# real-stanford/semantic-abstraction

Hardware: AMD Instinct MI355X
Metric: scenes/sec (relevancy+3D-UNet infer), 480x480x16-label x128^3 (higher is better)
Workload: dtype f16 (MFMA operands, fp32 accumulate; UNet hi/lo-split = fp32-equivalent); 1 GPU; end-to-end relevancy->fusion->OVSSC per scene: 480x480 RGB-D, 16 labels, ViT-B/16, 'ours' saliency config (2448 tile forwards), 128^3 voxels, 80000 input points; scene-sharded; arch=ViT-B/16, unet_precision=exact, tile_chunk_streams=1, scenes_per_gpu=26, parallelism=scene-shard x1, mode=throughput

## Files before the change

semantic-abstraction_amd/csrc/unet.hip:

```cpp
#include "semabs_common.h"

__device__ __forceinline__ int xcd_remap(int vb, int nb) {
    const int q = nb >> 3, r = nb & 7, x = vb & 7, k = vb >> 3;
    return (x < r ? x * (q + 1) : r * (q + 1) + (x - r) * q) + k;
}
__device__ __forceinline__ int xcd_persistent_tile(int vb, int G, int it, int total) {
    if (G & 7) { const long t = (long)it * G + vb; return t < total ? (int)t : -1; }
    const int x = vb & 7, j = vb >> 3, g8 = G >> 3;
    const int q = total >> 3, r = total & 7;
    const int lo = x < r ? x * (q + 1) : r * (q + 1) + (x - r) * q, cnt = q + (x < r ? 1 : 0);
    const long o = (long)it * g8 + j;
    return o < cnt ? lo + (int)o : -1;
}


template <int HID, int COUT>
__global__ __launch_bounds__(256, 2) void k_point_mlp(const float* __restrict__ xyz, const float* __restrict__ feat,
                                                   const float* __restrict__ w1, const float* __restrict__ b1,
                                                   const float* __restrict__ w2, const float* __restrict__ b2,
                                                   const float* __restrict__ w3, const float* __restrict__ b3,
                                                   float* __restrict__ out, int P, long N) {
    extern __shared__ __attribute__((aligned(16))) char smem[];
    float* sw2 = reinterpret_cast<float*>(smem);
    float* sw3 = sw2 + HID * HID;
// ... 901 lines not shown
    auto lds_barrier = [&]() { asm volatile("s_waitcnt lgkmcnt(0)\n\ts_barrier" ::: "memory"); };
    auto brick_of = [&](int it) { return xcd_persistent_tile((int)blockIdx.x, (int)gridDim.x, it, total); };
    if (producer) {
        int it = 0, brick = brick_of(0);
        if (brick >= 0) produce(brick, 0);
        lds_barrier();
        int buf = 0;
        for (; brick >= 0; buf ^= 1) {
            const int next = brick_of(++it);
            if (next >= 0 && !CONV16_ABL(a.ablate == 2 || a.ablate >= 4)) produce(next, buf ^ 1);
            lds_barrier();
            brick = next;
        }
    } else {
        load_weights();
        lds_barrier();
        int buf = 0, it = 0;
        for (int brick = brick_of(0); brick >= 0; brick = brick_of(++it), buf ^= 1) {
            if (!CONV16_ABL(a.ablate == 1)) consume(brick, buf);
            lds_barrier();
        }
        if (a.stats) flush_stats();
        if (GNB && a.gnb_bits) conv_absmax_commit(a.gnb_bits, amax);
    }
}

#define SEMABS_CONV_GENERIC 256
#define SEMABS_CONV_PACKED 512
#ifdef SEMABS_TUNING
static int g_conv16_ablate = 0;
static long long* g_conv_trace = nullptr;
static int g_brick_persist = 0;
static int g_convt_no_line = 0;
extern "C" int semabs_conv_tune(int key, long long value) {
    if (key == 0) g_conv16_ablate = (int)value & 7;
    else if (key == 1) g_conv_trace = reinterpret_cast<long long*>(value);
    else if (key == 2) g_brick_persist = (int)value;
    else if (key == 3) g_convt_no_line = (int)value;
    return SEMABS_OK;
}
#endif

static int conv16_lds_launch(const ConvArgs& a_in, int f32, hipStream_t s) {
    ConvArgs a = a_in;
#ifdef SEMABS_TUNING
    a.ablate = g_conv16_ablate;
#endif
    if (f32) {
        constexpr int T0 = 4;
        const size_t lds = (size_t)(((T0 + 2) * C16_H1 * C16_H2 * 8 + 127) / 128 * 128) * 2 * 2 * 2 * 2;
        const long total = (long)a.B * (a.I0 / T0) * (a.I1 / C16_T1) * (a.I2 / C16_T2);
        long nb = semabs_stream_cus(s); if (nb > total) nb = total;
        if (a.gnb_coef) {
            static SemabsLdsAttr attrg;
            semabs_ensure_lds(&k_conv16_lds<true, T0, true>, (int)(lds + 32 * 192), attrg);
            hipLaunchKernelGGL((k_conv16_lds<true, T0, true>), dim3((unsigned)nb), dim3(512), lds + (size_t)a.B * 192, s, a);
            SEMABS_CHECK_LAUNCH();
            return SEMABS_OK;
        }
        if (a.occ) {
            static SemabsLdsAttr attrs;
            semabs_ensure_lds(&k_conv16_lds<true, T0, false, true>, (int)lds, attrs);
            hipLaunchKernelGGL((k_conv16_lds<true, T0, false, true>), dim3((unsigned)nb), dim3(512), lds, s, a);
            SEMABS_CHECK_LAUNCH();
            return SEMABS_OK;
        }
        static SemabsLdsAttr attr;
        semabs_ensure_lds(&k_conv16_lds<true, T0>, (int)lds, attr);
        hipLaunchKernelGGL((k_conv16_lds<true, T0>), dim3((unsigned)nb), dim3(512), lds, s, a);
    } else {
        constexpr int T0 = 8;
// ... 349 lines not shown
    }
    BRICK_STAMP(7);
}

template <bool F32, int CW, int NB, bool ONE, bool PERSIST, int TX = 16, bool GNB = false>
static int conv_brick_launch_p(const ConvArgs& a, hipStream_t s) {
    const size_t lds = (size_t)((6 * C16_H1 * (TX + 2) * 8 + 127) / 128 * 128) * (CW / 8) * 2 * (F32 ? 2 : 1);
    static int per_cu = 0;
    if (!per_cu) {
        (void)hipFuncSetAttribute(reinterpret_cast<const void*>(&k_conv_brick<F32, CW, NB, ONE, PERSIST, TX, GNB>), hipFuncAttributeMaxDynamicSharedMemorySize, (int)lds);
        int n = 0;
        if (hipOccupancyMaxActiveBlocksPerMultiprocessor(&n, k_conv_brick<F32, CW, NB, ONE, PERSIST, TX, GNB>, 512, lds) != hipSuccess || n < 1) n = 1;
        per_cu = n;
    }
    const long total = (long)(a.I0 / 4) * (a.I1 / C16_T1) * (a.I2 / TX) * a.B * (a.Cout / (NB * 16));
    SEMABS_REQUIRE(total < (1L << 30), "conv brick: too many tiles");
    long nwg = total;
    if (PERSIST) { nwg = (long)semabs_stream_cus(s) * per_cu; if (nwg > total) nwg = total; }
    ConvArgs at = a;
#ifdef SEMABS_TUNING
    at.trace = g_conv_trace;
#endif
    hipLaunchKernelGGL((k_conv_brick<F32, CW, NB, ONE, PERSIST, TX, GNB>), dim3((unsigned)nwg), dim3(512), lds, s, at, (int)total);
    SEMABS_CHECK_LAUNCH();
    return SEMABS_OK;
}
template <bool F32, int CW, int NB, bool ONE>
static int conv_brick_launch_t(const ConvArgs& a, hipStream_t s) {
#ifdef SEMABS_TUNING
    if (g_brick_persist) return conv_brick_launch_p<F32, CW, NB, ONE, true>(a, s);
#endif
    return conv_brick_launch_p<F32, CW, NB, ONE, false>(a, s);
}
static int conv_brick_launch(const ConvArgs& a, int f32, hipStream_t s) {
    if (a.gnb_coef) {
        if (a.Cin == 32) return conv_brick_launch_p<true, 32, 2, true, false, 16, true>(a, s);
        return conv_brick_launch_p<true, 32, 2, false, false, 16, true>(a, s);
    }
    if (a.I2 % C16_T2 != 0) {
        return f32 ? conv_brick_launch_p<true, 32, 2, false, false, 8>(a, s) : conv_brick_launch_p<false, 32, 2, false, false, 8>(a, s);
    }
    const long bricks = (long)a.B * (a.I0 / 4) * (a.I1 / C16_T1) * (a.I2 / C16_T2);
    if (a.Cout == 16) {
        if (a.Cin == 32) return f32 ? conv_brick_launch_t<true, 32, 1, true>(a, s) : conv_brick_launch_t<false, 32, 1, true>(a, s);
        return f32 ? conv_brick_launch_t<true, 32, 1, false>(a, s) : conv_brick_launch_t<false, 32, 1, false>(a, s);
    }
    const bool nb4 = a.Cout % 64 == 0 && bricks * (a.Cout / 64) >= 512;
    if (a.Cin == 16) {
        if (nb4) return f32 ? conv_brick_launch_t<true, 16, 4, true>(a, s) : conv_brick_launch_t<false, 16, 4, true>(a, s);
        return f32 ? conv_brick_launch_t<true, 16, 2, true>(a, s) : conv_brick_launch_t<false, 16, 2, true>(a, s);
    }
    if (a.Cin == 32) {
        if (nb4) return f32 ? conv_brick_launch_t<true, 32, 4, true>(a, s) : conv_brick_launch_t<false, 32, 4, true>(a, s);
        return f32 ? conv_brick_launch_t<true, 32, 2, true>(a, s) : conv_brick_launch_t<false, 32, 2, true>(a, s);
    }
    if (nb4) return f32 ? conv_brick_launch_t<true, 32, 4, false>(a, s) : conv_brick_launch_t<false, 32, 4, false>(a, s);
    return f32 ? conv_brick_launch_t<true, 32, 2, false>(a, s) : conv_brick_launch_t<false, 32, 2, false>(a, s);
}

__global__ void k_conv_finish(float* __restrict__ y, const float* __restrict__ bias, const float* __restrict__ resid, long n4, int C, int relu) {
    const long i = (long)blockIdx.x * blockDim.x + threadIdx.x;
    if (i >= n4) return;
    float4 v = *reinterpret_cast<float4*>(y + i * 4);
    if (bias) { const float4 b = *reinterpret_cast<const float4*>(bias + (i * 4) % C); v.x += b.x; v.y += b.y; v.z += b.z; v.w += b.w; }
    if (resid) { const float4 r = *reinterpret_cast<const float4*>(resid + i * 4); v.x += r.x; v.y += r.y; v.z += r.z; v.w += r.w; }
    if (relu == 1) { v.x = fmaxf(v.x, 0.f); v.y = fmaxf(v.y, 0.f); v.z = fmaxf(v.z, 0.f); v.w = fmaxf(v.w, 0.f); }
    else if (relu == 2) { v.x = v.x > 0.f ? v.x : 0.01f * v.x; v.y = v.y > 0.f ? v.y : 0.01f * v.y; v.z = v.z > 0.f ? v.z : 0.01f * v.z; v.w = v.w > 0.f ? v.w : 0.01f * v.w; }
    *reinterpret_cast<float4*>(y + i * 4) = v;
}

static int conv_launch(const ConvArgs& a_in, int f32, hipStream_t s) {
    ConvArgs a = a_in;
    const long Mtot = (long)a.B * a.M0 * a.M1 * a.M2;
    a.ksplit = 1;
    if (f32 && a.os == 1 && a.Cout % 64 == 0 && a.Cin % 32 == 0 && a.ntaps == 27 && Mtot <= 16384) {
        const long slices = semabs_cdiv(Mtot, 4 * 32) * (a.Cout / 64);
        int ks = (int)(2048 / (slices > 0 ? slices : 1));
        if (ks > 27) ks = 27;
        if (ks >= 3) {
            a.ksplit = ks;
// ... 50 lines not shown
    const bool bricks = !(act_flags & SEMABS_CONV_GENERIC);
    int rc = conv_common_checks(x, w_hi, w_lo, y, Cin, Cout, act_f32);
    if (rc) return rc;
    SEMABS_REQUIRE(ksize == 1 || ksize == 3, "semabs_conv3d: kernel size must be 1 or 3");
    SEMABS_REQUIRE((gn_scale == nullptr) == (gn_shift == nullptr), "semabs_conv3d: gn_scale and gn_shift go together");
    ConvArgs a;
    a.x = x; a.y = y; a.w_hi = (const f16*)w_hi; a.w_lo = (const f16*)w_lo; a.gn_scale = gn_scale; a.gn_shift = gn_shift;
    a.bias = bias; a.resid = resid; a.B = B; a.I0 = D0; a.I1 = D1; a.I2 = D2; a.O0 = D0; a.O1 = D1; a.O2 = D2;
    a.M0 = D0; a.M1 = D1; a.M2 = D2; a.os = 1; a.is = 1; a.op0 = a.op1 = a.op2 = 0; a.Cin = Cin; a.Cout = Cout; a.relu = relu;
    a.ntaps = ksize * ksize * ksize;
    a.Kp = ((a.ntaps * Cin + 31) / 32) * 32;
    a.stats = nullptr; a.ablate = 0; a.trace = nullptr; a.wp_hi = nullptr; a.wp_lo = nullptr; a.ncls = 0;
    if (act_flags & SEMABS_CONV_PACKED) {
        a.wp_hi = a.w_hi + (long)Cout * a.Kp;
        if (w_lo) a.wp_lo = a.w_lo + (long)Cout * a.Kp;
    }
    int t = 0;
    for (int kd = 0; kd < ksize; ++kd)
        for (int kh = 0; kh < ksize; ++kh)
            for (int kw = 0; kw < ksize; ++kw, ++t) { a.td0[t] = kd - ksize / 2; a.td1[t] = kh - ksize / 2; a.td2[t] = kw - ksize / 2; }
    SEMABS_REQUIRE(relu == 0 || relu == 1 || (relu == 2 && ksize == 1), "semabs_conv3d: relu must be 0, 1, or 2 (LeakyReLU, ksize 1 only)");
    SEMABS_REQUIRE(!out_sums || (out_groups > 0 && Cout % out_groups == 0), "semabs_conv3d_stats: Cout must be a multiple of out_groups");
    bool fused = false;
    if (bricks && ksize == 3 && Cin == 16 && Cout == 16 && D0 % 8 == 0 && D1 % C16_T1 == 0 && D2 % C16_T2 == 0 && (long)D0 * D1 * D2 * 16 < (1L << 31)) {
        if (out_sums && out_groups == 8) { a.stats = out_sums; fused = true; }
        a.occ = occ;
        rc = conv16_lds_launch(a, act_f32, (hipStream_t)stream);
    } else if (occ) {
        semabs_set_error("semabs_conv3d_sparse_stats: the occupancy bitmap is read by the 16 -> 16 level-0 kernel only (D0 % 8, D1 % 8, D2 % 16 == 0)");
        return SEMABS_EINVAL;
    } else if (bricks && ksize == 3 && (Cout % 32 == 0 || (Cout == 16 && Cin % 32 == 0 && D2 % C16_T2 == 0)) && (Cin == 16 || Cin % 32 == 0) && relu != 2 &&
               D0 % 4 == 0 && D1 % C16_T1 == 0 && (D2 % C16_T2 == 0 || (D2 % 8 == 0 && Cin % 32 == 0))) {
        if (out_sums && out_groups == 8 && Cout >= 32) { a.stats = out_sums; fused = true; }
        rc = conv_brick_launch(a, act_f32, (hipStream_t)stream);
    } else {
        rc = conv_launch(a, act_f32, (hipStream_t)stream);
    }
    if (rc == SEMABS_OK && out_sums && !fused) rc = semabs_gn_stats(y, out_sums, B, (long)D0 * D1 * D2, Cout, out_groups, act_f32, stream);
    return rc;
}
extern "C" int semabs_conv3d(const void* x, const void* w_hi, const void* w_lo, void* y, const float* gn_scale, const float* gn_shift,
                             const float* bias, const void* resid, int B, int D0, int D1, int D2, int Cin, int Cout, int ksize,
                             int relu, int act_f32, void* stream) {
    return conv3d_impl(x, w_hi, w_lo, y, gn_scale, gn_shift, bias, resid, B, D0, D1, D2, Cin, Cout, ksize, relu, act_f32, nullptr, 0, stream);
}
extern "C" int semabs_conv3d_stats(const void* x, const void* w_hi, const void* w_lo, void* y, const float* gn_scale, const float* gn_shift,
                                   const float* bias, const void* resid, int B, int D0, int D1, int D2, int Cin, int Cout, int ksize,
                                   int relu, int act_f32, double* out_sums, int out_groups, void* stream) {
    SEMABS_REQUIRE(out_sums, "semabs_conv3d_stats: out_sums is null");
    return conv3d_impl(x, w_hi, w_lo, y, gn_scale, gn_shift, bias, resid, B, D0, D1, D2, Cin, Cout, ksize, relu, act_f32, out_sums, out_groups, stream);
}

extern "C" int semabs_conv3d_sparse_stats(const void* x, const unsigned int* occ, const void* w_hi, const void* w_lo, void* y, const float* gn_scale, const float* gn_shift,
                                          const float* bias, const void* resid, int B, int D0, int D1, int D2, int Cin, int Cout, int ksize,
                                          int relu, int act_f32, double* out_sums, int out_groups, void* stream) {
    SEMABS_REQUIRE(out_sums && occ, "semabs_conv3d_sparse_stats: out_sums / occ is null");
    SEMABS_REQUIRE(!(act_f32 & SEMABS_CONV_GENERIC), "semabs_conv3d_sparse_stats: the generic kernel reads the whole volume");
    return conv3d_impl(x, w_hi, w_lo, y, gn_scale, gn_shift, bias, resid, B, D0, D1, D2, Cin, Cout, ksize, relu, act_f32, out_sums, out_groups, stream, occ);
}

static int conv3d_gnbwd_route(int B, int D0, int D1, int D2, int Cin, int Cout, int G, bool have_add) {
    if (B <= 0 || G <= 0) return 0;
    if (B <= 32 && Cin == 16 && Cout == 16 && D0 % 8 == 0 && D1 % C16_T1 == 0 && D2 % C16_T2 == 0 && (long)D0 * D1 * D2 * 16 < (1L << 31) && 16 % G == 0) return 1;
    if (!have_add && Cin % 32 == 0 && Cout % 32 == 0 && Cout % G == 0 && (Cout / G) % 4 == 0 && D0 % 4 == 0 && D1 % C16_T1 == 0 && D2 % C16_T2 == 0) return 2;
    return 0;
}
extern "C" int semabs_conv3d_gnbwd_supported(int B, int D0, int D1, int D2, int Cin, int Cout, int G, int have_add1, int* ok) {
// ... 623 lines not shown
```

Baseline: 8.675 scenes/s.

## Add persistent warp-specialized producer/consumer conv kernel for wide-input fp32 UNet layers

Adds a new persistent 3D conv kernel in which four producer waves stage GroupNorm-applied, hi/lo-split f16 halo tiles into double-buffered LDS per 16-channel unit, while four consumer waves run MFMA with register-prefetched weights. For NB=2 it uses a dy-reuse schedule that shares each loaded input row across three kernel rows. It routes fp32 convs with Cin>=64 to it by default. The aim is to overlap global loads with MFMA and to cut redundant LDS and input traffic, at the cost of much more code, heavier register pressure and a new correctness surface.

```diff
diff --git a/semantic-abstraction_amd/csrc/unet.hip b/semantic-abstraction_amd/csrc/unet.hip
--- a/semantic-abstraction_amd/csrc/unet.hip
+++ b/semantic-abstraction_amd/csrc/unet.hip
@@ -957,11 +957,13 @@
 static long long* g_conv_trace = nullptr;
 static int g_brick_persist = 0;
 static int g_convt_no_line = 0;
+static int g_conv_units = 0;
 extern "C" int semabs_conv_tune(int key, long long value) {
     if (key == 0) g_conv16_ablate = (int)value & 7;
     else if (key == 1) g_conv_trace = reinterpret_cast<long long*>(value);
     else if (key == 2) g_brick_persist = (int)value;
     else if (key == 3) g_convt_no_line = (int)value;
+    else if (key == 4) g_conv_units = (int)value;
     return SEMABS_OK;
 }
 #endif
@@ -1377,6 +1379,408 @@
 #endif
     return conv_brick_launch_p<F32, CW, NB, ONE, false>(a, s);
 }
+
+template <int NB>
+__global__ __launch_bounds__(512) void k_conv_units(ConvArgs a, int total) {
+    constexpr bool DY = NB == 2;
+    constexpr int T0 = 4, H0 = T0 + 2, HX = C16_H2, HALO = H0 * C16_H1 * HX, NSTEPS = 14;
+    constexpr int PLANE = (HALO * 8 + 127) / 128 * 128;
+    constexpr int BUF_EL = PLANE * 2 * 2;
+    constexpr int ZPAD = HALO * 8;
+    static_assert(PLANE - ZPAD >= 8, "no room for the zero slot");
+    extern __shared__ __attribute__((aligned(16))) char smem[];
+    const int tid = threadIdx.x, lane = tid & 63;
+    const int wid = __builtin_amdgcn_readfirstlane(tid >> 6);
+    const int vl = lane & 15, kg = lane >> 4;
+    const int n2 = a.I2 / C16_T2, n1 = a.I1 / C16_T1, n0 = a.I0 / T0;
+    const int per_vol = n0 * n1 * n2;
+    const int Cin = a.Cin, U = Cin >> 4;
+    const bool has_gn = a.gn_scale != nullptr;
+    const bool producer = wid >= 4;
+    const int ptid = tid - 256;
+    float* const s_stat = reinterpret_cast<float*>(smem + (size_t)BUF_EL * 2 * 2);
+
+    auto tile_of = [&](int it) { return xcd_persistent_tile((int)blockIdx.x, (int)gridDim.x, it, total); };
+    auto decode = [&](int t, int& b, int& cout0, int& z0, int& y0, int& x0) {
+        int br = t % per_vol; t /= per_vol;
+        b = t % a.B; cout0 = (t / a.B) * (NB * 16);
+        const int t2 = br % n2; br /= n2;
+        const int t1 = br % n1; const int t0 = br / n1;
+        z0 = t0 * T0; y0 = t1 * C16_T1; x0 = t2 * C16_T2;
+    };
+    int my_tiles = 0;
+    while (tile_of(my_tiles) >= 0) ++my_tiles;
+    const int nunits = my_tiles * U;
+
+    if (tid < 32) {
+        f16x8 z;
+#pragma unroll
+        for (int e = 0; e < 8; ++e) z[e] = (f16)0.f;
+        *reinterpret_cast<f16x8*>(reinterpret_cast<f16*>(smem) + (tid >> 4) * BUF_EL + ((tid >> 3) & 1) * (PLANE * 2) + ZPAD + (tid & 7) * 8) = z;
+    }
+
+    auto produce = [&](int tile, int u, int buf) {
+        int b, cout0, z0, y0, x0;
+        decode(tile, b, cout0, z0, y0, x0);
+        f16* s_hi = reinterpret_cast<f16*>(smem) + buf * BUF_EL;
+        f16* s_lo = s_hi + PLANE * 2;
+        const int hsel = (ptid >> 3) & 1;
+        const int vsub = (ptid & 7) + ((ptid >> 4) << 3);
+        const int ch = u * 16 + hsel * 8;
+        float gs[8], gh[8];
+        if (has_gn) {
+            const float4* ps = reinterpret_cast<const float4*>(a.gn_scale + (long)b * Cin + ch);
+            const float4* pt = reinterpret_cast<const float4*>(a.gn_shift + (long)b * Cin + ch);
+            const float4 s0 = ps[0], s1 = ps[1], h0 = pt[0], h1 = pt[1];
+            gs[0] = s0.x; gs[1] = s0.y; gs[2] = s0.z; gs[3] = s0.w; gs[4] = s1.x; gs[5] = s1.y; gs[6] = s1.z; gs[7] = s1.w;
+            gh[0] = h0.x; gh[1] = h0.y; gh[2] = h0.z; gh[3] = h0.w; gh[4] = h1.x; gh[5] = h1.y; gh[6] = h1.z; gh[7] = h1.w;
+        } else {
+#pragma unroll
+            for (int j = 0; j < 8; ++j) { gs[j] = 1.f; gh[j] = 0.f; }
+        }
+        constexpr int NT = (HALO + 127) / 128;
+        const float* xb = reinterpret_cast<const float*>(a.x) + (size_t)b * a.I0 * a.I1 * a.I2 * Cin;
+        float raw[NT][8];
+        bool inb[NT];
+#pragma unroll
+        for (int k = 0; k < NT; ++k) {
+            const int v = min(vsub + k * 128, HALO - 1);
+            const int hx = v % HX, hy = (v / HX) % C16_H1, hz = v / (HX * C16_H1);
+            const int gz = z0 + hz - 1, gy = y0 + hy - 1, gx = x0 + hx - 1;
+            inb[k] = gz >= 0 && gz < a.I0 && gy >= 0 && gy < a.I1 && gx >= 0 && gx < a.I2;
+            const int cz = min(max(gz, 0), a.I0 - 1), cy = min(max(gy, 0), a.I1 - 1), cx = min(max(gx, 0), a.I2 - 1);
+            const unsigned eo = (unsigned)(((cz * a.I1 + cy) * a.I2 + cx) * Cin + ch);
+            const float4 q0 = *reinterpret_cast<const float4*>(xb + eo), q1 = *reinterpret_cast<const float4*>(xb + eo + 4);
+            raw[k][0] = q0.x; raw[k][1] = q0.y; raw[k][2] = q0.z; raw[k][3] = q0.w; raw[k][4] = q1.x; raw[k][5] = q1.y; raw[k][6] = q1.z; raw[k][7] = q1.w;
+        }
+#pragma unroll
+        for (int k = 0; k < NT; ++k) {
+            const int v = vsub + k * 128;
+            f16x8 h, l;
+#pragma unroll
+            for (int c = 0; c < 8; ++c) {
+                const float val = inb[k] ? raw[k][c] * gs[c] + gh[c] : 0.f;
+                h[c] = (f16)val;
+                l[c] = (f16)(val - (float)h[c]);
+            }
+            if (v < HALO) {
+                *reinterpret_cast<f16x8*>(s_hi + hsel * PLANE + v * 8) = h;
+                *reinterpret_cast<f16x8*>(s_lo + hsel * PLANE + v * 8) = l;
+            }
+        }
+    };
+
+    auto lds_barrier = [&]() { asm volatile("s_waitcnt lgkmcnt(0)\n\ts_barrier" ::: "memory"); };
+    if (producer) {
+        if (nunits > 0) produce(tile_of(0), 0, 0);
+        lds_barrier();
+        int it = 0, u = 0;
+#pragma unroll 1
+        for (int n = 0; n < nunits; ++n) {
+            if (++u == U) { u = 0; ++it; }
+            if (n + 1 < nunits) produce(tile_of(it), u, (n + 1) & 1);
+            lds_barrier();
+        }
+        lds_barrier();
+        return;
+    }
+
+    const bool packed = a.wp_hi != nullptr;
+    const int ncb = a.Cout >> 4;
+    const f16* const wbase_h = packed ? a.wp_hi : a.w_hi;
+    const f16* const wbase_l = packed ? a.wp_lo : a.w_lo;
+    const int wnb = packed ? 512 : 16 * a.Kp;
+    auto w_index = [&](int ks, int u, int cout0, int kgl, int vll) -> int {
+        const int half = kgl & 1, tsel = kgl >> 1, vl = vll;
+        const int ka = 2 * ks * Cin + u * 16, kb = min(2 * ks + 1, 26) * Cin + u * 16;
+        const int k = (tsel ? kb : ka) + half * 8;
+        return packed ? (((k >> 5) * ncb + (cout0 >> 4)) * 64 + ((k >> 3) & 3) * 16 + vl) * 8 : (cout0 + vl) * a.Kp + k;
+    };
+    auto geom = [&](int ks, int& xo, int& rs, int kgl, int vll) {
+        const int half = kgl & 1, tsel = kgl >> 1;
+        const int rb = ((wid + 1) * C16_H1 + 1) * HX + (vll + 1);
+        const int ta = 2 * ks, tb = min(2 * ks + 1, 26);
+        const int offa = ((ta / 9) - 1) * C16_H1 * HX + (((ta / 3) % 3) - 1) * HX + ((ta % 3) - 1);
+        const int offb = ((tb / 9) - 1) * C16_H1 * HX + (((tb / 3) % 3) - 1) * HX + ((tb % 3) - 1);
+        const bool dead = tsel && ks == NSTEPS - 1;
+        xo = dead ? ZPAD : half * PLANE + (rb + (tsel ? offb : offa)) * 8;
+        rs = dead ? 0 : HX * 8;
+    };
+    const int v2 = lane >> 2, k2 = lane & 3;
+    int st_b = 0, st_c = 0, st_set = 0;
+    bool pend = false;
+    auto flush_stats = [&]() {
+        if (wid == 0) {
+            const int cg = a.Cout >> 3;
+            const int spg = min(cg >> 2, NB * 4);
+            if (lane < (NB * 4 / spg) * 2) {
+                const int g = lane >> 1, m = lane & 1;
+                double sum = 0.0;
+                for (int w = 0; w < 4; ++w)
+                    for (int sl = 0; sl < spg; ++sl) sum += (double)s_stat[(((st_set * 4 + w) * NB * 4) + g * spg + sl) * 2 + m];
+                atomicAdd(a.stats + ((long)st_b * 8 + st_c / cg + g) * 2 + m, sum);
+            }
+        }
+        pend = false;
+    };
+
+    f32x4 acc[8][NB];
+    f16x8 wa_h[NB], wa_l[NB], wb_h[NB], wb_l[NB];
+    auto load_w = [&](int widx, f16x8* wh, f16x8* wl) {
+#pragma unroll
+        for (int nb = 0; nb < NB; ++nb) {
+            wh[nb] = *reinterpret_cast<const f16x8*>(wbase_h + widx + nb * wnb);
+            wl[nb] = *reinterpret_cast<const f16x8*>(wbase_l + widx + nb * wnb);
+        }
+    };
+    auto w_index_dy = [&](int st, int dy, int u, int cout0, int kgl, int vll) -> int {
+        const int tsel_cin = (kgl >> 1) ? Cin : 0, half = kgl & 1, vl = vll;
+        const int qa = 2 * st, qb = 2 * st + 1 < 9 ? 2 * st + 1 : qa;
+        const int tapa = (qa / 3) * 9 + dy * 3 + (qa % 3), tapb = (qb / 3) * 9 + dy * 3 + (qb % 3);
+        const int k = (tapa * Cin + u * 16) + ((tapb - tapa) * tsel_cin + half * 8);
+        return packed ? (((k >> 5) * ncb + (cout0 >> 4)) * 64 + ((k >> 3) & 3) * 16 + vl) * 8 : (cout0 + vl) * a.Kp + k;
+    };
+    f16x8 wc_h[3][NB], wc_l[3][NB], wn_h[3][NB], wn_l[3][NB];
+    auto load_w_dy = [&](int st, int u, int cout0, f16x8 (*wh)[NB], f16x8 (*wl)[NB], int kgl, int vll) {
+#pragma unroll
+        for (int dy = 0; dy < 3; ++dy) {
+            const int widx = w_index_dy(st, dy, u, cout0, kgl, vll);
+#pragma unroll
+            for (int nb = 0; nb < NB; ++nb) {
+                wh[dy][nb] = *reinterpret_cast<const f16x8*>(wbase_h + widx + nb * wnb);
+                wl[dy][nb] = *reinterpret_cast<const f16x8*>(wbase_l + widx + nb * wnb);
+            }
+        }
+    };
+    if (my_tiles > 0) {
+        const int c0 = (tile_of(0) / (per_vol * a.B)) * (NB * 16);
+        if constexpr (DY) load_w_dy(0, 0, c0, wc_h, wc_l, kg, vl);
+        else load_w(w_index(0, 0, c0, kg, vl), wa_h, wa_l);
+    }
+    lds_barrier();
+    int n = 0;
+#pragma unroll 1
+    for (int it = 0; it < my_tiles; ++it) {
+        int b, cout0, z0, y0, x0;
+        decode(tile_of(it), b, cout0, z0, y0, x0);
+        const int ncout0 = it + 1 < my_tiles ? (tile_of(it + 1) / (per_vol * a.B)) * (NB * 16) : cout0;
+#pragma unroll
+        for (int r = 0; r < 8; ++r)
+#pragma unroll
+            for (int nb = 0; nb < NB; ++nb) acc[r][nb] = f32x4{0.f, 0.f, 0.f, 0.f};
+#pragma unroll 1
+        for (int u = 0; u < U; ++u, ++n) {
+            const f16* const sb_hi = reinterpret_cast<const f16*>(smem) + (n & 1) * BUF_EL;
+            const f16* const sb_lo = sb_hi + PLANE * 2;
+            const int nx_u = u + 1 < U ? u + 1 : 0, nx_c = u + 1 < U ? cout0 : ncout0;
+            if constexpr (DY) {
+                int kgl = kg, vll = vl;
+                asm volatile("" : "+v"(kgl), "+v"(vll));
+                int xbase[5];
+                const int fb = (kgl & 1) * PLANE + (wid * C16_H1 * HX + vll) * 8;
+#pragma unroll
+                for (int st = 0; st < 5; ++st) {
+                    const int qa = 2 * st, qb = 2 * st + 1 < 9 ? 2 * st + 1 : qa;
+                    const int q = (kgl >> 1) ? qb : qa;
+                    xbase[st] = fb + ((q / 3) * C16_H1 * HX + (q % 3)) * 8;
+                }
+                const int rs4 = (kgl >> 1) ? 0 : HX * 8;
+                if (kgl >> 1) xbase[4] = ZPAD;
+                f16x8 xh[3], xl[3];
+                constexpr int RHO[10] = {2, 0, 3, 1, 4, 9, 5, 8, 6, 7};
+                auto request = [&](int i, int slot) {
+                    const int st = i / 10, rho = RHO[i % 10];
+                    const int off = xbase[st] + rho * (st == 4 ? rs4 : HX * 8);
+                    xh[slot] = *reinterpret_cast<const f16x8*>(sb_hi + off);
+                    xl[slot] = *reinterpret_cast<const f16x8*>(sb_lo + off);
+                };
+                request(0, 0);
+                request(1, 1);
+                __builtin_amdgcn_sched_barrier(0);
+#pragma unroll
+                for (int st = 0; st < 5; ++st) {
+                    load_w_dy(st < 4 ? st + 1 : 0, st < 4 ? u : nx_u, st < 4 ? cout0 : nx_c, wn_h, wn_l, kgl, vll);
+                    __builtin_amdgcn_sched_barrier(0);
+#pragma unroll
+                    for (int ri = 0; ri < 10; ++ri) {
+                        const int i = st * 10 + ri, slot = i % 3, rho = RHO[ri];
+                        bool first = true;
+#pragma unroll
+                        for (int kind = 0; kind < 3; ++kind) {
+#pragma unroll
+                            for (int dy = 0; dy < 3; ++dy) {
+                                const int r = rho - dy;
+                                if (r < 0 || r >= 8) continue;
+#pragma unroll
+                                for (int nb = 0; nb < NB; ++nb) {
+                                    acc[r][nb] = __builtin_amdgcn_mfma_f32_16x16x32_f16(kind == 1 ? wc_l[dy][nb] : wc_h[dy][nb], kind == 2 ? xl[slot] : xh[slot], acc[r][nb], 0, 0, 0);
+                                    if (first) {
+                                        first = false;
+                                        if (i + 2 < 50) request(i + 2, (i + 2) % 3);
+                                        __builtin_amdgcn_sched_barrier(0);
+                                    }
+                                }
+                            }
+                        }
+                        __builtin_amdgcn_sched_barrier(0);
+                    }
+#pragma unroll
+                    for (int dy = 0; dy < 3; ++dy)
+#pragma unroll
+                        for (int nb = 0; nb < NB; ++nb) { wc_h[dy][nb] = wn_h[dy][nb]; wc_l[dy][nb] = wn_l[dy][nb]; }
+                }
+                lds_barrier();
+                if (pend) flush_stats();
+                continue;
+            }
+            int kgl = kg, vll = vl;
+            asm volatile("" : "+v"(kgl), "+v"(vll));
+            f16x8 xh[4], xl[4];
+            auto step = [&](int ks, int ksn, int un, int cn, f16x8* wh, f16x8* wl, f16x8* whn, f16x8* wln) {
+                int xo, rs, xon, rsn;
+                geom(ks, xo, rs, kgl, vll);
+                geom(ksn, xon, rsn, kgl, vll);
+                const int wn = w_index(ksn, un, cn, kgl, vll);
+                if (whn) load_w(wn, whn, wln);
+                __builtin_amdgcn_sched_barrier(0);
+#pragma unroll
+                for (int hh = 0; hh < 2; ++hh) {
+                    const int xo2 = hh == 0 ? xo + 4 * rs : xon, rs2 = hh == 0 ? rs : rsn;
+#pragma unroll
+                    for (int nb = 0; nb < NB; ++nb) {
+                        const bool lastb = nb == NB - 1;
+#pragma unroll
+                        for (int r = 0; r < 4; ++r)
+                            acc[hh * 4 + r][nb] = __builtin_amdgcn_mfma_f32_16x16x32_f16(wh[nb], xh[r], acc[hh * 4 + r][nb], 0, 0, 0);
+#pragma unroll
+                        for (int r = 0; r < 4; ++r) {
+                            acc[hh * 4 + r][nb] = __builtin_amdgcn_mfma_f32_16x16x32_f16(wl[nb], xh[r], acc[hh * 4 + r][nb], 0, 0, 0);
+                            if (lastb) { xh[r] = *reinterpret_cast<const f16x8*>(sb_hi + xo2 + r * rs2); __builtin_amdgcn_sched_barrier(0); }
+                        }
+#pragma unroll
+                        for (int r = 0; r < 4; ++r) {
+                            acc[hh * 4 + r][nb] = __builtin_amdgcn_mfma_f32_16x16x32_f16(wh[nb], xl[r], acc[hh * 4 + r][nb], 0, 0, 0);
+                            if (lastb) { xl[r] = *reinterpret_cast<const f16x8*>(sb_lo + xo2 + r * rs2); __builtin_amdgcn_sched_barrier(0); }
+                        }
+                        if (!whn && hh == 1) {
+                            __builtin_amdgcn_sched_barrier(0);
+                            wh[nb] = *reinterpret_cast<const f16x8*>(wbase_h + wn + nb * wnb);
+                            wl[nb] = *reinterpret_cast<const f16x8*>(wbase_l + wn + nb * wnb);
+                            __builtin_amdgcn_sched_barrier(0);
+                        }
+                    }
+                }
+                __builtin_amdgcn_sched_barrier(0);
+            };
+            {
+                int xo, rs;
+                geom(0, xo, rs, kgl, vll);
+#pragma unroll
+                for (int r = 0; r < 4; ++r) {
+                    xh[r] = *reinterpret_cast<const f16x8*>(sb_hi + xo + r * rs);
+                    xl[r] = *reinterpret_cast<const f16x8*>(sb_lo + xo + r * rs);
+                }
+            }
+            if constexpr (NB <= 2) {
+#pragma unroll 1
+                for (int ks = 0; ks < NSTEPS; ks += 2) {
+                    const bool last = ks + 2 >= NSTEPS;
+                    step(ks, ks + 1, u, cout0, wa_h, wa_l, wb_h, wb_l);
+                    step(ks + 1, last ? 0 : ks + 2, last ? nx_u : u, last ? nx_c : cout0, wb_h, wb_l, wa_h, wa_l);
+                }
+            } else {
+#pragma unroll 1
+                for (int ks = 0; ks < NSTEPS; ++ks) {
+                    const bool last = ks + 1 >= NSTEPS;
+                    step(ks, last ? 0 : ks + 1, last ? nx_u : u, last ? nx_c : cout0, wa_h, wa_l, nullptr, nullptr);
+                }
+            }
+            lds_barrier();
+            if (pend) flush_stats();
+        }
+        {
+            const int src = (k2 * 16 + v2) << 2;
+            float st_s[NB], st_q[NB];
+#pragma unroll
+            for (int nb = 0; nb < NB; ++nb) { st_s[nb] = 0.f; st_q[nb] = 0.f; }
+            constexpr int RG = (NB == 4 || DY) ? 4 : 8;
+            const long orow0 = ((((long)b * a.I0 + (z0 + wid)) * a.I1 + y0) * a.I2 + (x0 + v2)) * a.Cout + (cout0 + 4 * k2);
+            const long orow = (long)a.I2 * a.Cout;
+#pragma unroll
+            for (int g = 0; g < 8 / RG; ++g) {
+                float q[RG][NB][4];
+#pragma unroll
+                for (int r = 0; r < RG; ++r)
+#pragma unroll
+                    for (int nb = 0; nb < NB; ++nb) {
+                        if (a.resid) {
+                            const float4 t = *reinterpret_cast<const float4*>(reinterpret_cast<const float*>(a.resid) + orow0 + (g * RG + r) * orow + nb * 16);
+                            q[r][nb][0] = t.x; q[r][nb][1] = t.y; q[r][nb][2] = t.z; q[r][nb][3] = t.w;
+                        } else {
+                            q[r][nb][0] = q[r][nb][1] = q[r][nb][2] = q[r][nb][3] = 0.f;
+                        }
+                    }
+                __builtin_amdgcn_sched_barrier(0);
+#pragma unroll
+                for (int r = 0; r < RG; ++r)
+#pragma unroll
+                    for (int nb = 0; nb < NB; ++nb) {
+                        const int rr = g * RG + r;
+                        const float a0 = acc[rr][nb][0], a1 = acc[rr][nb][1], a2 = acc[rr][nb][2], a3 = acc[rr][nb][3];
+                        float o[4];
+                        o[0] = __int_as_float(__builtin_amdgcn_ds_bpermute(src, __float_as_int(a0)));
+                        o[1] = __int_as_float(__builtin_amdgcn_ds_bpermute(src, __float_as_int(a1)));
+                        o[2] = __int_as_float(__builtin_amdgcn_ds_bpermute(src, __float_as_int(a2)));
+                        o[3] = __int_as_float(__builtin_amdgcn_ds_bpermute(src, __float_as_int(a3)));
+#pragma unroll
+                        for (int j = 0; j < 4; ++j) o[j] += q[r][nb][j];
+                        if (a.bias) { const float4 bv = *reinterpret_cast<const float4*>(a.bias + cout0 + nb * 16 + 4 * k2); o[0] += bv.x; o[1] += bv.y; o[2] += bv.z; o[3] += bv.w; }
+                        if (a.relu) { o[0] = fmaxf(o[0], 0.f); o[1] = fmaxf(o[1], 0.f); o[2] = fmaxf(o[2], 0.f); o[3] = fmaxf(o[3], 0.f); }
+                        *reinterpret_cast<float4*>(reinterpret_cast<float*>(a.y) + orow0 + rr * orow + nb * 16) = make_float4(o[0], o[1], o[2], o[3]);
+                        st_s[nb] += (o[0] + o[1]) + (o[2] + o[3]);
+                        st_q[nb] += (o[0] * o[0] + o[1] * o[1]) + (o[2] * o[2] + o[3] * o[3]);
+                    }
+            }
+            if (a.stats) {
+#pragma unroll
+                for (int nb = 0; nb < NB; ++nb) {
+                    float vs = st_s[nb], vq = st_q[nb];
+#pragma unroll
+                    for (int m = 4; m < 64; m <<= 1) { vs += __shfl_xor(vs, m, 64); vq += __shfl_xor(vq, m, 64); }
+                    if (v2 == 0) {
+                        float* p = s_stat + ((((it & 1) * 4 + wid) * NB * 4) + nb * 4 + k2) * 2;
+                        p[0] = vs; p[1] = vq;
+                    }
+                }
+                st_b = b; st_c = cout0; st_set = it & 1; pend = true;
+            }
+        }
+    }
+    lds_barrier();
+    if (pend) flush_stats();
+}
+
+template <int NB>
+static int conv_units_launch(const ConvArgs& a, hipStream_t s) {
+    const size_t lds = (size_t)((6 * C16_H1 * C16_H2 * 8 + 127) / 128 * 128) * 2 * 2 * 2 * 2 + 2 * 4 * NB * 4 * 2 * sizeof(float);
+    const long total = (long)(a.I0 / 4) * (a.I1 / C16_T1) * (a.I2 / C16_T2) * a.B * (a.Cout / (NB * 16));
+    SEMABS_REQUIRE(total < (1L << 30), "conv units: too many tiles");
+    long nwg = semabs_stream_cus(s); if (nwg > total) nwg = total;
+    static SemabsLdsAttr attr;
+    semabs_ensure_lds(&k_conv_units<NB>, (int)lds, attr);
+    hipLaunchKernelGGL((k_conv_units<NB>), dim3((unsigned)nwg), dim3(512), lds, s, a, (int)total);
+    SEMABS_CHECK_LAUNCH();
+    return SEMABS_OK;
+}
+static bool conv_units_route(const ConvArgs& a) {
+    if (!(a.Cin == 16 || a.Cin == 32 || a.Cin == 64 || a.Cin == 128)) return false;
+    if ((long)a.I0 * a.I1 * a.I2 * a.Cin >= (1L << 31) || (long)a.Cout * a.Kp >= (1L << 28)) return false;
+#ifdef SEMABS_TUNING
+    if (g_conv_units == 1) return false;
+    if (g_conv_units == 2) return true;
+#endif
+    return a.Cin >= 64;
+}
 static int conv_brick_launch(const ConvArgs& a, int f32, hipStream_t s) {
     if (a.gnb_coef) {
         if (a.Cin == 32) return conv_brick_launch_p<true, 32, 2, true, false, 16, true>(a, s);
@@ -1391,6 +1795,7 @@
         return f32 ? conv_brick_launch_t<true, 32, 1, false>(a, s) : conv_brick_launch_t<false, 32, 1, false>(a, s);
     }
     const bool nb4 = a.Cout % 64 == 0 && bricks * (a.Cout / 64) >= 512;
+    if (f32 && conv_units_route(a)) return nb4 ? conv_units_launch<4>(a, s) : conv_units_launch<2>(a, s);
     if (a.Cin == 16) {
         if (nb4) return f32 ? conv_brick_launch_t<true, 16, 4, true>(a, s) : conv_brick_launch_t<false, 16, 4, true>(a, s);
         return f32 ? conv_brick_launch_t<true, 16, 2, true>(a, s) : conv_brick_launch_t<false, 16, 2, true>(a, s);
```

After: 8.694 scenes/s, median of 6. Within noise of the previous version (+0.2%).

## Add persistent double-buffered brick conv kernel streaming channel-chunk units

Applied to the files above, without the earlier changes.

Adds a persistent 3D conv kernel, k_conv_brick_units. Each workgroup walks (tile, channel-chunk) units in an XCD-aware order. The next unit's halo is prefetched from global memory during the current unit's MFMA k-loop, then committed into a second LDS buffer. Weights are double-buffered in registers, and the epilogue fuses residual, bias, ReLU and GroupNorm stats. By default it handles fp32-activation convs with Cin >= 64, aiming to hide global load latency and cut launch and tail overhead. The cost is a heavier register footprint and a larger LDS footprint per workgroup, with a grid capped at one workgroup per CU.

```diff
diff --git a/semantic-abstraction_amd/csrc/unet.hip b/semantic-abstraction_amd/csrc/unet.hip
--- a/semantic-abstraction_amd/csrc/unet.hip
+++ b/semantic-abstraction_amd/csrc/unet.hip
@@ -1377,7 +1377,293 @@
 #endif
     return conv_brick_launch_p<F32, CW, NB, ONE, false>(a, s);
 }
-static int conv_brick_launch(const ConvArgs& a, int f32, hipStream_t s) {
+template <int NB, bool ONE>
+__global__ __launch_bounds__(512) void k_conv_brick_units(ConvArgs a, int total) {
+    constexpr int T0 = 4, H0 = T0 + 2, TX = 16, HX = TX + 2, HALO = H0 * C16_H1 * HX, NTHR = 512;
+    constexpr int R = 4, CW = 16, CPV = CW / 8, NSTEPS = 14;
+    constexpr int PLANE = (HALO * 8 + 127) / 128 * 128;
+    constexpr int UNIT = PLANE * CPV * 2;
+    constexpr int ZOFF = HALO * 8;
+    extern __shared__ __attribute__((aligned(16))) char smem[];
+    f16* const s_buf = reinterpret_cast<f16*>(smem);
+    float* const s_stat = reinterpret_cast<float*>(s_buf + 2 * UNIT);
+    const int tid = threadIdx.x, lane = tid & 63;
+    const int wid = __builtin_amdgcn_readfirstlane(tid >> 6);
+    const int vl = lane & 15, kg = lane >> 4;
+    const int n2 = a.I2 / TX, n1 = a.I1 / C16_T1, n0 = a.I0 / T0;
+    const int per_vol = n0 * n1 * n2;
+    const bool has_gn = a.gn_scale != nullptr;
+    const int Cin = ONE ? CW : a.Cin;
+    const int nchunks = ONE ? 1 : Cin / CW;
+    const int ncb = a.Cout >> 4;
+    auto lds_barrier = [&]() { asm volatile("s_waitcnt lgkmcnt(0)\n\ts_barrier" ::: "memory"); };
+    auto tile_of = [&](int it) { return xcd_persistent_tile((int)blockIdx.x, (int)gridDim.x, it, total); };
+    auto decode = [&](int t, int& b, int& cout0, int& z0, int& y0, int& x0) {
+        int br = t % per_vol; t /= per_vol;
+        b = t % a.B; cout0 = (t / a.B) * (NB * 16);
+        const int t2 = br % n2; br /= n2;
+        const int t1 = br % n1; const int t0 = br / n1;
+        z0 = t0 * T0; y0 = t1 * C16_T1; x0 = t2 * TX;
+    };
+    int rbase[R];
+#pragma unroll
+    for (int r = 0; r < R; ++r) {
+        const int f = wid * R + r;
+        rbase[r] = (((f >> 3) + 1) * C16_H1 + ((f & 7) + 1)) * HX + (vl + 1);
+    }
+    constexpr int VPI = NTHR / CPV, NIT = (HALO + VPI - 1) / VPI;
+    const int c = tid % CPV, vsub = tid / CPV;
+    float raw[NIT][8];
+    float gs[8], gh[8];
+    unsigned inb = 0;
+    auto issue = [&](int tile, int cc) {
+        int b, cout0, z0, y0, x0;
+        decode(tile, b, cout0, z0, y0, x0);
+        const int ch = cc * CW + c * 8;
+        if (has_gn) {
+            const float4* ps = reinterpret_cast<const float4*>(a.gn_scale + (long)b * Cin + ch);
+            const float4* pt = reinterpret_cast<const float4*>(a.gn_shift + (long)b * Cin + ch);
+            const float4 s0 = ps[0], s1 = ps[1], h0 = pt[0], h1 = pt[1];
+            gs[0] = s0.x; gs[1] = s0.y; gs[2] = s0.z; gs[3] = s0.w; gs[4] = s1.x; gs[5] = s1.y; gs[6] = s1.z; gs[7] = s1.w;
+            gh[0] = h0.x; gh[1] = h0.y; gh[2] = h0.z; gh[3] = h0.w; gh[4] = h1.x; gh[5] = h1.y; gh[6] = h1.z; gh[7] = h1.w;
+        } else {
+#pragma unroll
+            for (int j = 0; j < 8; ++j) { gs[j] = 1.f; gh[j] = 0.f; }
+        }
+        inb = 0;
+#pragma unroll
+        for (int it = 0; it < NIT; ++it) {
+            const int v = min(vsub + it * VPI, HALO - 1);
+            const int hx = v % HX, hy = (v / HX) % C16_H1, hz = v / (HX * C16_H1);
+            const int gz = z0 + hz - 1, gy = y0 + hy - 1, gx = x0 + hx - 1;
+            if (gz >= 0 && gz < a.I0 && gy >= 0 && gy < a.I1 && gx >= 0 && gx < a.I2) inb |= 1u << it;
+            const int cz = min(max(gz, 0), a.I0 - 1), cy = min(max(gy, 0), a.I1 - 1), cx = min(max(gx, 0), a.I2 - 1);
+            load8<true>(a.x, ((((long)b * a.I0 + cz) * a.I1 + cy) * a.I2 + cx) * Cin + ch, raw[it]);
+        }
+    };
+    auto commit = [&](int buf) {
+        f16* const s_hi = s_buf + buf * UNIT;
+#pragma unroll
+        for (int it = 0; it < NIT; ++it) {
+            const int v = vsub + it * VPI;
+            const bool in = (inb >> it) & 1u;
+            f16x8 h, l;
+#pragma unroll
+            for (int j = 0; j < 8; ++j) {
+                const float val = in ? raw[it][j] * gs[j] + gh[j] : 0.f;
+                h[j] = (f16)val; l[j] = (f16)(val - (float)h[j]);
+            }
+            if (v < HALO) {
+                const int off = c * PLANE + v * 8;
+                *reinterpret_cast<f16x8*>(s_hi + off) = h;
+                *reinterpret_cast<f16x8*>(s_hi + CPV * PLANE + off) = l;
+            }
+        }
+    };
+    f32x4 acc[R][NB];
+    auto zero_acc = [&]() {
+#pragma unroll
+        for (int r = 0; r < R; ++r)
+#pragma unroll
+            for (int nb = 0; nb < NB; ++nb) acc[r][nb] = f32x4{0.f, 0.f, 0.f, 0.f};
+    };
+    auto kloop = [&](int cc, int buf, int cout0, auto prefetch) {
+        const f16* const s_hi = s_buf + buf * UNIT;
+        auto x_off = [&](int ks, int* off) {
+            const int ta = 2 * ks, tb = (2 * ks + 1 < 27) ? 2 * ks + 1 : 26;
+            const int offa = ((ta / 9) - 1) * C16_H1 * HX + (((ta / 3) % 3) - 1) * HX + ((ta % 3) - 1);
+            const int offb = ((tb / 9) - 1) * C16_H1 * HX + (((tb / 3) % 3) - 1) * HX + ((tb % 3) - 1);
+            const int voff = (kg >> 1) ? offb : offa;
+            const bool dead = !ONE && ks == NSTEPS - 1 && (kg >> 1);
+#pragma unroll
+            for (int r = 0; r < R; ++r) off[r] = dead ? ZOFF - buf * UNIT : (kg & 1) * PLANE + (rbase[r] + voff) * 8;
+        };
+        auto w_index = [&](int ks, int nb) -> long {
+            const int tap = ONE ? 2 * ks + (kg >> 1) : min(2 * ks + (kg >> 1), 26);
+            const int k = tap * Cin + cc * CW + (kg & 1) * 8;
+            return ((long)((k >> 5) * ncb + (cout0 >> 4) + nb) * 64 + ((k >> 3) & 3) * 16 + vl) * 8;
+        };
+        auto load_w = [&](int ks, f16x8* wh, f16x8* wl) {
+#pragma unroll
+            for (int nb = 0; nb < NB; ++nb) {
+                const long widx = w_index(ks, nb);
+                wh[nb] = *reinterpret_cast<const f16x8*>(a.wp_hi + widx);
+                wl[nb] = *reinterpret_cast<const f16x8*>(a.wp_lo + widx);
+            }
+        };
+        f16x8 xh[R], xl[R];
+        auto step = [&](int ks, f16x8* wh, f16x8* wl, f16x8* whn, f16x8* wln, auto mid) {
+            const int ksn = ks + 1 < NSTEPS ? ks + 1 : ks;
+            int offn[R];
+            x_off(ksn, offn);
+            if (whn) { load_w(ksn, whn, wln); mid(); }
+            __builtin_amdgcn_sched_barrier(0);
+#pragma unroll
+            for (int nb = 0; nb < NB; ++nb) {
+                const bool lastb = nb == NB - 1;
+#pragma unroll
+                for (int r = 0; r < R; ++r) acc[r][nb] = __builtin_amdgcn_mfma_f32_16x16x32_f16(wh[nb], xh[r], acc[r][nb], 0, 0, 0);
+#pragma unroll
+                for (int r = 0; r < R; ++r) {
+                    acc[r][nb] = __builtin_amdgcn_mfma_f32_16x16x32_f16(wl[nb], xh[r], acc[r][nb], 0, 0, 0);
+                    if (lastb) { xh[r] = *reinterpret_cast<const f16x8*>(s_hi + offn[r]); __builtin_amdgcn_sched_barrier(0); }
+                }
+#pragma unroll
+                for (int r = 0; r < R; ++r) {
+                    acc[r][nb] = __builtin_amdgcn_mfma_f32_16x16x32_f16(wh[nb], xl[r], acc[r][nb], 0, 0, 0);
+                    if (lastb) { xl[r] = *reinterpret_cast<const f16x8*>(s_hi + CPV * PLANE + offn[r]); __builtin_amdgcn_sched_barrier(0); }
+                }
+                if (!whn) {
+                    __builtin_amdgcn_sched_barrier(0);
+                    const long widx = w_index(ksn, nb);
+                    wh[nb] = *reinterpret_cast<const f16x8*>(a.wp_hi + widx);
+                    wl[nb] = *reinterpret_cast<const f16x8*>(a.wp_lo + widx);
+                    __builtin_amdgcn_sched_barrier(0);
+                }
+            }
+            if (!whn) mid();
+            __builtin_amdgcn_sched_barrier(0);
+        };
+        auto nothing = []() {};
+        {
+            int off0[R];
+            x_off(0, off0);
+#pragma unroll
+            for (int r = 0; r < R; ++r) {
+                xh[r] = *reinterpret_cast<const f16x8*>(s_hi + off0[r]);
+                xl[r] = *reinterpret_cast<const f16x8*>(s_hi + CPV * PLANE + off0[r]);
+            }
+        }
+        if constexpr (NB <= 2) {
+            f16x8 wa_h[NB], wa_l[NB], wb_h[NB], wb_l[NB];
+            load_w(0, wa_h, wa_l);
+            step(0, wa_h, wa_l, wb_h, wb_l, prefetch);
+            step(1, wb_h, wb_l, wa_h, wa_l, nothing);
+#pragma unroll 1
+            for (int ks = 2; ks < NSTEPS; ks += 2) {
+                step(ks, wa_h, wa_l, wb_h, wb_l, nothing);
+                step(ks + 1, wb_h, wb_l, wa_h, wa_l, nothing);
+            }
+        } else {
+            f16x8 wh[NB], wl[NB];
+            load_w(0, wh, wl);
+            step(0, wh, wl, nullptr, nullptr, prefetch);
+#pragma unroll 1
+            for (int ks = 1; ks < NSTEPS; ++ks) step(ks, wh, wl, nullptr, nullptr, nothing);
+        }
+    };
+    auto epilogue = [&](int tile) {
+        int b, cout0, z0, y0, x0;
+        decode(tile, b, cout0, z0, y0, x0);
+        const int v2 = lane >> 2, k2 = lane & 3;
+        const int src = (k2 * 16 + v2) << 2;
+        long obase[R];
+        float q[R][NB][4];
+        float st_s[NB], st_q[NB];
+#pragma unroll
+        for (int nb = 0; nb < NB; ++nb) { st_s[nb] = 0.f; st_q[nb] = 0.f; }
+#pragma unroll
+        for (int r = 0; r < R; ++r) {
+            const int f = wid * R + r;
+            const long ovox = (((long)b * a.I0 + (z0 + (f >> 3))) * a.I1 + (y0 + (f & 7))) * a.I2 + (x0 + v2);
+            obase[r] = ovox * a.Cout + (cout0 + 4 * k2);
+#pragma unroll
+            for (int nb = 0; nb < NB; ++nb) {
+                if (a.resid) {
+                    const float4 t = *reinterpret_cast<const float4*>(reinterpret_cast<const float*>(a.resid) + obase[r] + nb * 16);
+                    q[r][nb][0] = t.x; q[r][nb][1] = t.y; q[r][nb][2] = t.z; q[r][nb][3] = t.w;
+                } else {
+                    q[r][nb][0] = q[r][nb][1] = q[r][nb][2] = q[r][nb][3] = 0.f;
+                }
+            }
+        }
+        __builtin_amdgcn_sched_barrier(0);
+#pragma unroll
+        for (int r = 0; r < R; ++r) {
+#pragma unroll
+            for (int nb = 0; nb < NB; ++nb) {
+                const int co = cout0 + nb * 16 + 4 * k2;
+                const float a0 = acc[r][nb][0], a1 = acc[r][nb][1], a2 = acc[r][nb][2], a3 = acc[r][nb][3];
+                float o[4];
+                o[0] = __int_as_float(__builtin_amdgcn_ds_bpermute(src, __float_as_int(a0)));
+                o[1] = __int_as_float(__builtin_amdgcn_ds_bpermute(src, __float_as_int(a1)));
+                o[2] = __int_as_float(__builtin_amdgcn_ds_bpermute(src, __float_as_int(a2)));
+                o[3] = __int_as_float(__builtin_amdgcn_ds_bpermute(src, __float_as_int(a3)));
+#pragma unroll
+                for (int j = 0; j < 4; ++j) o[j] += q[r][nb][j];
+                if (a.bias) { const float4 bv = *reinterpret_cast<const float4*>(a.bias + co); o[0] += bv.x; o[1] += bv.y; o[2] += bv.z; o[3] += bv.w; }
+                if (a.relu) { o[0] = fmaxf(o[0], 0.f); o[1] = fmaxf(o[1], 0.f); o[2] = fmaxf(o[2], 0.f); o[3] = fmaxf(o[3], 0.f); }
+                *reinterpret_cast<float4*>(reinterpret_cast<float*>(a.y) + obase[r] + nb * 16) = make_float4(o[0], o[1], o[2], o[3]);
+                st_s[nb] += (o[0] + o[1]) + (o[2] + o[3]);
+                st_q[nb] += (o[0] * o[0] + o[1] * o[1]) + (o[2] * o[2] + o[3] * o[3]);
+            }
+        }
+        if (a.stats) {
+            const int cg = a.Cout >> 3;
+#pragma unroll
+            for (int nb = 0; nb < NB; ++nb) {
+                float vs = st_s[nb], vq = st_q[nb];
+#pragma unroll
+                for (int m = 4; m < 64; m <<= 1) { vs += __shfl_xor(vs, m, 64); vq += __shfl_xor(vq, m, 64); }
+                if (v2 == 0) {
+                    const int gl = (nb * 16 + 4 * k2) / cg;
+                    atomicAdd(&s_stat[gl * 2], vs); atomicAdd(&s_stat[gl * 2 + 1], vq);
+                }
+            }
+            lds_barrier();
+            const int ngl = (NB * 16 >= cg) ? NB * 16 / cg : 1;
+            if (tid < ngl * 2) {
+                atomicAdd(a.stats + ((long)b * 8 + cout0 / cg + (tid >> 1)) * 2 + (tid & 1), (double)s_stat[tid]);
+                s_stat[tid] = 0.f;
+            }
+        }
+    };
+
+    int it = 0, tile = tile_of(0);
+    if (tile < 0) return;
+    if (tid < 16) s_stat[tid] = 0.f;
+    if (tid < 16) {
+        reinterpret_cast<unsigned*>(s_buf + ZOFF)[tid] = 0u;
+        reinterpret_cast<unsigned*>(s_buf + CPV * PLANE + ZOFF)[tid] = 0u;
+    }
+    issue(tile, 0);
+    commit(0);
+    lds_barrier();
+    zero_acc();
+    for (int cc = 0, buf = 0;; buf ^= 1) {
+        int ntile = tile, ncc = cc + 1;
+        if (ncc == nchunks) { ncc = 0; ntile = tile_of(++it); }
+        const bool more = ntile >= 0;
+        kloop(cc, buf, (tile / (per_vol * a.B)) * (NB * 16), [&]() { if (more) issue(ntile, ncc); });
+        if (more) commit(buf ^ 1);
+        lds_barrier();
+        if (ncc == 0) { epilogue(tile); zero_acc(); }
+        if (!more) break;
+        tile = ntile; cc = ncc;
+    }
+}
+
+#define SEMABS_CONV_BRICK_SEQ 1024
+#define SEMABS_CONV_WIDE 2048
+#define SEMABS_CONV_UNITS 4096
+#define SEMABS_CONV_GRID(flags) (((flags) >> 16) & 0xfff)
+template <int NB, bool ONE>
+static int conv_brick_units_launch(const ConvArgs& a, int flags, hipStream_t s) {
+    constexpr int PLANE = (6 * C16_H1 * 18 * 8 + 127) / 128 * 128;
+    constexpr int lds = PLANE * 2 * 2 * 2 * 2 + 64;
+    static SemabsLdsAttr attr;
+    semabs_ensure_lds(&k_conv_brick_units<NB, ONE>, lds, attr);
+    const long total = (long)(a.I0 / 4) * (a.I1 / C16_T1) * (a.I2 / C16_T2) * a.B * (a.Cout / (NB * 16));
+    SEMABS_REQUIRE(total < (1L << 30), "conv brick: too many tiles");
+    long nwg = semabs_stream_cus(s);
+    if (SEMABS_CONV_GRID(flags) && SEMABS_CONV_GRID(flags) < nwg) nwg = SEMABS_CONV_GRID(flags);
+    if (nwg > total) nwg = total;
+    hipLaunchKernelGGL((k_conv_brick_units<NB, ONE>), dim3((unsigned)nwg), dim3(512), (size_t)lds, s, a, (int)total);
+    SEMABS_CHECK_LAUNCH();
+    return SEMABS_OK;
+}
+
+static int conv_brick_launch(const ConvArgs& a, int f32, hipStream_t s, int flags = 0) {
     if (a.gnb_coef) {
         if (a.Cin == 32) return conv_brick_launch_p<true, 32, 2, true, false, 16, true>(a, s);
         return conv_brick_launch_p<true, 32, 2, false, false, 16, true>(a, s);
@@ -1390,7 +1676,12 @@
         if (a.Cin == 32) return f32 ? conv_brick_launch_t<true, 32, 1, true>(a, s) : conv_brick_launch_t<false, 32, 1, true>(a, s);
         return f32 ? conv_brick_launch_t<true, 32, 1, false>(a, s) : conv_brick_launch_t<false, 32, 1, false>(a, s);
     }
-    const bool nb4 = a.Cout % 64 == 0 && bricks * (a.Cout / 64) >= 512;
+    const bool nb4 = a.Cout % 64 == 0 && (bricks * (a.Cout / 64) >= 512 || (flags & SEMABS_CONV_WIDE));
+    if (f32 && a.wp_hi && a.wp_lo && !(flags & SEMABS_CONV_BRICK_SEQ) && (a.Cin >= 64 || (flags & SEMABS_CONV_UNITS))) {
+        const bool w4 = a.Cout % 64 == 0 && (a.Cin >= 64 || nb4);
+        if (a.Cin == 16) return w4 ? conv_brick_units_launch<4, true>(a, flags, s) : conv_brick_units_launch<2, true>(a, flags, s);
+        return w4 ? conv_brick_units_launch<4, false>(a, flags, s) : conv_brick_units_launch<2, false>(a, flags, s);
+    }
     if (a.Cin == 16) {
         if (nb4) return f32 ? conv_brick_launch_t<true, 16, 4, true>(a, s) : conv_brick_launch_t<false, 16, 4, true>(a, s);
         return f32 ? conv_brick_launch_t<true, 16, 2, true>(a, s) : conv_brick_launch_t<false, 16, 2, true>(a, s);
@@ -1507,7 +1798,7 @@
     } else if (bricks && ksize == 3 && (Cout % 32 == 0 || (Cout == 16 && Cin % 32 == 0 && D2 % C16_T2 == 0)) && (Cin == 16 || Cin % 32 == 0) && relu != 2 &&
                D0 % 4 == 0 && D1 % C16_T1 == 0 && (D2 % C16_T2 == 0 || (D2 % 8 == 0 && Cin % 32 == 0))) {
         if (out_sums && out_groups == 8 && Cout >= 32) { a.stats = out_sums; fused = true; }
-        rc = conv_brick_launch(a, act_f32, (hipStream_t)stream);
+        rc = conv_brick_launch(a, act_f32, (hipStream_t)stream, act_flags);
     } else {
         rc = conv_launch(a, act_f32, (hipStream_t)stream);
     }
```

Result: no change. 8.444 scenes/s before, 8.418 scenes/s after (-0.3%).
